# sasg/cilium

Hardware: AMD Instinct MI355X
Metric: classified headers/sec (Mpps, whole node) at 100k-prefix ipcache + 16k-ID policy (higher is better)
Workload: dtype u32

## Files before the change

### cilium_amd/csrc/cfc_api.cpp

```cpp
#include <hip/hip_runtime.h>

#include <algorithm>
#include <cerrno>
#include <cstdio>
#include <cstdlib>
#include <cstring>
#include <map>
#include <set>
#include <memory>
#include <mutex>
#include <string>
#include <thread>
#include <unordered_set>
#include <type_traits>
#include <vector>

#include "../../include/cfc.h"
#include "classify.hpp"
#include "selfcut.hpp"
#include "ctmirror.hpp"
#include "flatten.hpp"
#include "maps.hpp"

using namespace cfc;
// ... 1719 lines not shown
    r.ep = ep_lxc;
    r.m = m;
    const size_t tb = nat_sort_tmp_bytes(m);
    const size_t m4 = 4ull * ((m + 3) & ~3u);
    const size_t rows = V6 ? 5 * m4 + m4 : 8 * m4 + 4 * m4 + m4;
    if (r.idx.ensure(4ull * m) || c->nat_tmp.ensure(tb) || r.rows.ensure(rows) ||
        r.outs.ensure(3 * m4 + 2 * m4))
        return -ENOMEM;
    uint32_t *idx = (uint32_t *)r.idx.p;
    if (int rc = nat_sort((const uint32_t *)c->nat_list.p, idx, m, in.n, c->nat_tmp.p, tb, s))
        return rc;
    char *rp = (char *)r.rows.p, *op = (char *)r.outs.p;
    r.o = cfc_out{};
    r.o.verdict = (int32_t *)op;
    r.o.identity = (uint32_t *)(op + m4);
    r.o.notify = out.notify ? (uint32_t *)(op + 2 * m4) : nullptr;
    r.o.action = (uint8_t *)(op + 3 * m4);
    r.o.ct = (uint8_t *)(op + 4 * m4);
    EgressArgs e2 = ea;
    e2.nat_idx = e2.nat_cnt = nullptr;
    e2.sums = nullptr;
    e2.svo = nullptr;
    const int smode = V6 ? CFC_MODE_EGRESS : CFC_MODE_INGRESS;
    const WsLayout wl = ws_layout(m, T, smode, true);
    if (r.ws.ensure(wl.total))
        return -ENOMEM;
    DevTables Th = T;
    Th.ct_sum = nullptr;
    int rc;
    if constexpr (V6) {
        NatHop4 h{};
        h.sa = (uint32_t *)rp;
        h.da = (uint32_t *)(rp + m4);
        h.pt = (uint32_t *)(rp + 2 * m4);
        h.mt = (uint32_t *)(rp + 3 * m4);
        h.hash = T.lb4 ? (uint32_t *)(rp + 4 * m4) : nullptr;
        h.tf = (uint8_t *)(rp + 5 * m4);
        r.h4 = cfc_hdr_v4{h.sa, h.da, h.pt, h.mt, nullptr, h.tf, m, h.hash};
        rc = nat64_gather(in, idx, m, ea.nat_v4, h, s);
        uint32_t nsvo = 0;
        if (!rc && T.lb4) {
            const size_t sb = svc_order_tmp_bytes(m);
            if (c->svo_keys.bytes < 8ull * m || c->svo.bytes < 4ull * m ||
                c->svo_tmp.bytes < sb) {
                (void)hipStreamSynchronize(s);
                if (c->svo_keys.ensure(8ull * m) || c->svo_keys2.ensure(8ull * m) ||
                    c->svo_tmp.ensure(sb) || c->svo.zeros(4ull * m, s))
// ... 10 lines not shown
                e2.svo = (const uint32_t *)c->svo.p;
        }
        if (!rc)
            rc = launch_classify_v4(Th, r.h4, r.o, smode, e2, c->ctr, (uint32_t *)r.ws.p,
                                    c->num_cus, s, nullptr);
        if ((nsvo || (rc && T.lb4)) && c->svo.p &&
            hipMemsetAsync(c->svo.p, 0, 4ull * m, s) != hipSuccess && !rc)
            rc = -EIO;
    } else {
        NatHop6 h{};
        h.sa = (uint4 *)rp;
        h.da = (uint4 *)(rp + 4 * m4);
        h.pt = (uint32_t *)(rp + 8 * m4);
        h.mt = (uint32_t *)(rp + 9 * m4);
        h.mk = (uint32_t *)(rp + 10 * m4);
        h.id = (uint32_t *)(rp + 11 * m4);
        h.tf = (uint8_t *)(rp + 12 * m4);
        r.h6 = cfc_hdr_v6{(const uint8_t *)h.sa, (const uint8_t *)h.da, h.pt, h.mt, h.mk, h.tf,
                          m, nullptr};
        e2.nat_id = h.id;
        const bool egr = mode == CFC_MODE_EGRESS;
        cfc_hdr_v4 gin = in;
        if (egr && (T.lb4 || T.rnat4)) {
            const WsLayout lw = ws_layout(in.n, T, mode, true);
            const uint32_t *a = (const uint32_t *)((const char *)c->ws + lw.lb);
            const uint64_t st = (in.n + 3) & ~3ull;
            gin.saddr = a + 2 * st;
            gin.daddr = a + 3 * st;
        }
        rc = nat46_gather(T, gin, egr ? nullptr : out.identity, ea.seclabel, idx, m,
                          (const uint4 *)c->epoch->ep->nat6.p, h, s);
        if (!rc)
            rc = launch_classify_v6(Th, r.h6, r.o, smode, e2, c->ctr, (uint32_t *)r.ws.p,
                                    c->num_cus, s, nullptr);
    }
    if (!rc)
        rc = nat_scatter(idx, m, r.o, out, !V6 && mode == CFC_MODE_EGRESS, s);
    c->n_nat_hops += m;
    if (rc || !out.ct)
        r.family = 0;
    return rc;
}

struct Launch4 {
    const uint32_t *tr_id = nullptr;
    int operator()(const DevTables &T, const cfc_hdr_v4 &in, const cfc_out &out, int mode,
                   const EgressArgs &E, uint64_t *ctr, uint32_t *ws, int cus, hipStream_t s,
// ... 49 lines not shown
        if (mode == CFC_MODE_EGRESS) {
            auto it = E.ep->nat4.find(ep_lxc);
            ea.nat_v4 = it == E.ep->nat4.end() ? 0u : it->second;
            nat_list = ea.nat_v4 != 0 && in->n;
        }
    } else {
        T.nat46 = mode != CFC_MODE_XDP && E.T.ct4 && E.ep->nat6.p &&
                  (E.ct->n_nat46 || c->nat46_seen);
        nat_list = T.nat46 && in->n;
    }
    if (nat_list) {
        if (c->nat_list.bytes < 4 * in->n) {
            (void)hipStreamSynchronize(s);
            if (c->nat_list.ensure(4 * in->n))
                return -ENOMEM;
        }
        if (c->nat_cnt.ensure(16) || hipMemsetAsync(c->nat_cnt.p, 0, 4, s) != hipSuccess)
            return -ENOMEM;
        ea.nat_idx = (uint32_t *)c->nat_list.p;
        ea.nat_cnt = (uint32_t *)c->nat_cnt.p;
    }
    const WsLayout wl = ws_layout(in->n, E.T, mode,
                                  E.T.ct4 || E.T.ct6 || out->ct || E.T.lb4 || E.T.rnat4 ||
                                      E.T.lb6 || E.T.rnat6);
    const size_t need = wl.total;
    c->last_cls.valid = false;
    if (need > c->ws_bytes) {
        if (c->ws) {
            (void)hipDeviceSynchronize();
            (void)hipFree(c->ws);
        }
        c->ws = nullptr;
        c->ws_bytes = 0;
        if (hipMalloc((void **)&c->ws, need) != hipSuccess)
            return -ENOMEM;
        c->ws_bytes = need;
    }
    if (c->ctr_pending && c->last_stream != s)
        (void)hipStreamWaitEvent(s, c->last_done, 0);
    order_after_launches(c, s);
    uint32_t nsvo = 0;
    if (mode == CFC_MODE_EGRESS && in->n &&
        (std::is_same<Hdr, cfc_hdr_v6>::value ? E.T.lb6 != nullptr : E.T.lb4 != nullptr)) {
        const uint64_t n = in->n;
        const size_t tb = svc_order_tmp_bytes(n);
        if (c->svo_keys.bytes < 8 * n || c->svo.bytes < 4 * n || c->svo_tmp.bytes < tb) {
            (void)hipStreamSynchronize(s);
// ... 2551 lines not shown
```

### cilium_amd/csrc/classify.hip

```cpp
#include <algorithm>
#include <cstdlib>
#include <mutex>
#include <set>
#include <tuple>
#include <vector>

#include "kern_common.hpp"
#ifndef CFC_EXP
#define CFC_EXP 0
#endif

namespace cfc {

namespace {

constexpr int LDS_MET_U64 = 18;
template <int MODE>
constexpr int met_n()
{
    return MODE == CFC_MODE_EGRESS ? 7 : MODE == CFC_MODE_XDP ? 0 : 4;
}
template <int MODE>
constexpr int acc_n()
{
// ... 500 lines not shown
    p.lxc_slots = (T.lxc4 && T.lxc4_lds) ? T.lxc4_mask + 1 : 0;
    p.pf_words = T.pf_bloom ? T.pf_bloom_words : 0;
    p.pol_words = T.pol_bloom ? T.pol_bloom_words : 0;
    p.pol_disp = T.pol_direct ? p.pol_words : 0;
    return p;
}

template <int MODE>
__device__ __forceinline__ void acc_publish(const unsigned long long *s_met,
                                            const CountArgs &C, uint32_t seclabel)
{
    for (uint32_t j = threadIdx.x; j < 2u * acc_n<MODE>(); j += BLOCK) {
        const unsigned long long v = s_met[j];
        if (!v)
            continue;
        const uint32_t k = j >> 1;
        uint64_t *dst = k < (uint32_t)met_n<MODE>()
                            ? C.g_met + met_reason_dir<MODE>(k) * 2
                            : C.g_id + id_index(ID_DIR_INGRESS, seclabel, k - met_n<MODE>());
        atomicAdd((unsigned long long *)dst + (j & 1), v);
    }
}

template <int MODE, int U, bool CT, bool NT, bool OPT, bool LB, int FAST, bool TR = false>
__global__ __launch_bounds__(BLOCK, WAVES_PER_SIMD) void k_classify_v4(
    DevTables T, LdsPlan L, cfc_hdr_v4 in, cfc_out out, EgressArgs E,
    CountArgs C, uint64_t per_block, LbIn LI, const uint32_t *tr_id)
{
    if (FAST) {
        T.tbl24 = T.tbl8 = T.pf_tbl24 = T.pf_tbl8 = nullptr;
        T.l4_shift = 32 - FAST;
        __builtin_assume(T.l4d != nullptr);
        __builtin_assume(T.lxc4 != nullptr);
        if (MODE == CFC_MODE_XDP || MODE == CFC_MODE_FULL)
            __builtin_assume(T.pf_fix != nullptr);
    }
    unsigned long long *s_met = lds_met();
    Lds S;
    S.lxc_off = LDS_MET_U64 / 2;
    const uint32_t pf4 = S.lxc_off + L.lxc_slots;
    const uint32_t pol4 = pf4 + L.pf_words / 4;
    S.pfb_off = 4 * pf4;
    S.polb_off = 4 * pol4;
    S.lxc = FAST || L.lxc_slots != 0;
    S.pfb = FAST || L.pf_words != 0;
    S.polb = FAST || L.pol_words != 0;
// ... 31 lines not shown
        if (out.ct)
            out.ct += start;
    }
    out.verdict += start;
    out.identity += start;
    if (out.notify)
        out.notify += start;
    constexpr bool LBE = LB && MODE == CFC_MODE_EGRESS;
    if (LBE) {
        LI.tda += start;
        LI.tpt += start;
        LI.psa += start;
        LI.fl += start;
    }
    if (LB && out.pkt_saddr) {
        out.pkt_saddr += start;
        out.pkt_daddr += start;
        out.pkt_ports += start;
    }
    if (C.ct)
        C.ct += start;
    if (C.ct2)
        C.ct2 += start;
    if (C.ctr)
        C.ctr += start;
    if (C.ctr2)
        C.ctr2 += start;
    if (C.id)
        C.id += start;
    if (TR)
        tr_id += start;
    MetAcc<acc_n<MODE>()> acc;
    acc.clear();
    uint32_t iter = 0;
    Raw nx[U];
#pragma unroll
    for (int u = 0; u < U; u++)
        r1_issue<OPT, LBE>(in, LI, u * BLOCK + threadIdx.x, end, nx[u]);
    for (uint32_t base = 0; base < end; base += BLOCK * U) {
        Hdr h[U];
#pragma unroll
        for (int u = 0; u < U; u++)
            r1_take(nx[u], base + u * BLOCK + threadIdx.x, end, h[u]);
#pragma unroll
        for (int u = 0; u < U; u++)
            r2_issue<MODE>(T, S, h[u]);
#pragma unroll
        for (int u = 0; u < U; u++)
            r3_identity<MODE, CT, LB, TR>(T, S, E, h[u], tr_id,
                                          min(base + u * BLOCK + threadIdx.x, end - 1));
        const uint32_t nb = base + BLOCK * U;
#pragma unroll
// ... 13 lines not shown
                if (OPT && out.action)
                    sto((uint8_t)h[u].act, out.action, o);
                if (CT && OPT && out.ct)
                    sto((uint8_t)h[u].ct_byte, out.ct, o);
                if (NT)
                    sto_nt((uint32_t)(h[u].ver < 0
                              ? notify_word(MODE, h[u].ver,
                                            EGR && h[u].met1 == mkey<MODE>(DROP_POLICY, METRIC_INGRESS),
                                            h[u].rec.w & 0xFFFF, E.lxc_id)
                              : h[u].evw),
                          out.notify, o4);
                if (CT) {
                    sto_nt(h[u].ct_k1, C.ct, o4);
                    if (EGR)
                        sto_nt(h[u].ct_k2, C.ct2, o4);
                }
                if (LB && out.pkt_saddr) {
                    sto_nt(h[u].psa, out.pkt_saddr, o4);
                    sto_nt(h[u].da, out.pkt_daddr, o4);
                    sto_nt(h[u].ppt, out.pkt_ports, o4);
                }
                if (MODE != CFC_MODE_XDP) {
#if CFC_EXP != 3
                    sto_nt(ctr_key(C, h[u].ctr0, len), C.ctr, o4);
#endif
                    if (EGR)
                        sto_nt(ctr_key(C, h[u].ctr1, len), C.ctr2, o4);
#if CFC_EXP != 3
                    sto_nt(h[u].idw, C.id, o4);
#endif
                }
            }
            if (WL && E.wbits) {
                bool pr;
                const bool w = wl_want<EGR>(h[u].ct_byte, h[u].ver, h[u].mt, h[u].ct_k1,
                                            EGR ? h[u].ct_k2 : NONE, pr);
                const uint64_t wb = __ballot(w && h[u].valid), pb = __ballot(pr && h[u].valid);
                const uint32_t w0 = base + u * BLOCK + (threadIdx.x & ~63u);
                if ((threadIdx.x & 63) == 0 && w0 < end) {
                    E.wbits[(start + w0) >> 6] = wb;
                    E.wprobe[(start + w0) >> 6] = pb;
                }
            }
            if (MODE != CFC_MODE_XDP && E.nat_idx)
                list_append(E.nat_idx, E.nat_cnt, h[u].nat && h[u].valid, (uint32_t)start + i);
            if (MODE != CFC_MODE_XDP && h[u].valid && h[u].id_ovf && h[u].need_pol)
                id_count(C, id_dir, h[u].ident, h[u].drop1, len);
            if (LBE && h[u].valid && h[u].ver == DROP_NO_SERVICE) {
                unsigned long long *m = reinterpret_cast<unsigned long long *>(
                    C.g_met + (uint64_t)(-DROP_NO_SERVICE * METRIC_DIRS + METRIC_EGRESS) * 2);
                atomicAdd(m, 1ull);
                atomicAdd(m + 1, (unsigned long long)len);
            }
#if CFC_EXP != 5
            acc.add(h[u].valid ? h[u].met0 : NONE, len);
#endif
            if (EGR) {
                acc.add(h[u].valid ? h[u].met1 : NONE, len);
                acc.add(h[u].valid && h[u].ev2 ? met_n<MODE>() + h[u].ev2 - 1 : NONE, len);
            }
        }
        if (++iter == 65536 / (2 * U)) {
            acc.flush(s_met);
            iter = 0;
        }
    }
    acc.flush(s_met);
    __syncthreads();
    acc_publish<MODE>(s_met, C, E.seclabel);
}

}

namespace {

struct HistJob {
    const uint32_t *keys;
    uint64_t poff;
    uint32_t lo, cnt;
    uint32_t kind;
    uint32_t packed;
};
constexpr int HIST_JOBS_MAX = 12;
struct HistJobs {
    HistJob j[HIST_JOBS_MAX];
};
constexpr uint64_t SLICE_MAX = 1ull << 31;

__device__ __forceinline__ unsigned long long *hist_dst(const HistJob &jb, uint32_t key,
                                                        uint64_t *g_ctr, uint64_t *g_id,
                                                        uint32_t id_dir)
{
    return reinterpret_cast<unsigned long long *>(
        jb.kind == 0 ? g_ctr + 2ull * key : g_id + id_index(id_dir, key >> 1, key & 1));
}

struct HistLds {
    uint32_t *ek, *ec, *ew;
    uint32_t *s;
};
__device__ __forceinline__ HistLds hist_lds()
{
    uint32_t *b = reinterpret_cast<uint32_t *>(cfc_smem);
    return HistLds{b, b + HIST_ESC_SLOTS, b + 2 * HIST_ESC_SLOTS, b + 3 * HIST_ESC_SLOTS};
// ... 35 lines not shown
    uint32_t h = fmix32(a.r) & (HIST_ESC_SLOTS - 1);
    for (int p = 0; p < 8; p++) {
        uint32_t cur = L.ek[h];
        if (cur == NONE) {
            cur = atomicCAS(&L.ek[h], NONE, a.r);
            if (cur == NONE)
                cur = a.r;
        }
        if (cur == a.r) {
            if (carry)
                atomicAdd(&L.ec[h], carry);
            if (wrap)
                atomicAdd(&L.ew[h], wrap);
            return;
        }
        h = (h + 1) & (HIST_ESC_SLOTS - 1);
    }
    unsigned long long *d = hist_dst(jb, jb.lo + a.r, g_ctr, g_id, id_dir);
    atomicAdd(d, (unsigned long long)HistSlot::esc_packets(carry, wrap));
    if (carry)
        atomicAdd(d + 1, (unsigned long long)HistSlot::esc_bytes(carry));
}

__global__ __launch_bounds__(BLOCK) void k_hist(HistJobs J, const uint32_t *meta,
                                                uint64_t n, uint64_t per_block,
                                                uint32_t *partial, uint64_t *g_ctr,
                                                uint64_t *g_id, uint32_t id_dir)
{
    const HistJob jb = J.j[blockIdx.y];
    const HistLds L = hist_lds();
    uint32_t *s = L.s;
    for (uint32_t j = threadIdx.x; j < HIST_ESC_SLOTS; j += BLOCK) {
        L.ek[j] = NONE;
        L.ec[j] = 0;
        L.ew[j] = 0;
    }
    for (uint32_t j = threadIdx.x; j < jb.cnt; j += BLOCK)
        s[j] = 0;
    __syncthreads();
    const uint64_t start = (uint64_t)blockIdx.x * per_block;
    const uint64_t end = min(n, start + per_block);
    const uint64_t end4 = start + ((end - start) & ~3ull);
    const bool meta16 = (reinterpret_cast<uintptr_t>(meta) & 15) == 0;
    auto load = [&](uint64_t i, uint4 &w, uint4 &m) {
        w = make_uint4(KEY_NONE, KEY_NONE, KEY_NONE, KEY_NONE);
        m = make_uint4(0, 0, 0, 0);
        if (i >= end4)
            return;
        w = ld_nt4(jb.keys + i);
        if (!jb.packed) {
            if (meta16) {
                m = ld_nt4(meta + i);
            } else {
                m.x = meta[i];
                m.y = meta[i + 1];
                m.z = meta[i + 2];
                m.w = meta[i + 3];
            }
        }
    };
    const uint64_t i0 = start + 4 * threadIdx.x;
    uint4 w0, m0, w1, m1;
    load(i0, w0, m0);
    load(i0 + 4 * BLOCK, w1, m1);
// ... 742 lines not shown
    hipLaunchKernelGGL(k_patch16, dim3((unsigned)((n + 255) / 256)), dim3(256), 0, s, rec, n);
    return hipGetLastError() == hipSuccess ? 0 : -5;
}

int launch_add_u64(uint64_t *dst, const uint64_t *src, uint64_t n,
                   hipStream_t s)
{
    if (!n)
        return 0;
    hipLaunchKernelGGL(k_add_u64, dim3((unsigned)((n + 255) / 256)), dim3(256),
                       0, s, dst, src, n);
    return hipGetLastError() == hipSuccess ? 0 : -5;
}

uint32_t ctp_buckets(const DevTables &T)
{
    if (getenv("CFC_ACC_PER_SLICE"))
        return 0;
    const uint64_t slots = (T.ct4 ? T.ct4_mask + 1ull : 0) + (T.ct6 ? T.ct6_mask + 1ull : 0);
    const uint64_t nb = (2 * slots + CTP_BUCKET - 1) / CTP_BUCKET;
    return nb <= CTP_MAX_BUCKETS ? (uint32_t)nb : 0u;
}

WsLayout ws_layout(uint64_t n, const DevTables &T, int mode, bool ct)
{
    WsLayout w{};
    if (n == 0 || mode == CFC_MODE_XDP)
        return w;
    const bool egr = mode == CFC_MODE_EGRESS;
    const size_t a = 4 * ctr_stride(n);
    size_t off = 0;
    w.ctr = off;
    off += a;
    if (egr) {
        w.ctr2 = off;
        off += a;
    }
    w.id = off;
    off += a;
    if (ct) {
        w.ct = off;
        off += a;
        if (egr) {
            w.ct2 = off;
            off += a;
        }
    }
    off = (off + 255) & ~(size_t)255;
    w.partial = off;
    const uint64_t slots = hist_slots(T, mode);
    w.nblk = hist_slices(n, slots);
    off += 4ull * slots * w.nblk;
    const uint32_t nbuck = ctp_buckets(T);
    if (ct && T.ct_st && nbuck) {
        const uint64_t per = acc_slice(n);
        const uint32_t nblk = (uint32_t)((n + per - 1) / per);
        w.ctp_nv = nblk * (egr ? 2u : 1u);
        w.ctp_nbuck = nbuck;
        w.ctp_nco = (nbuck + ACC_FINE - 1) / ACC_FINE;
        const uint64_t cap = (uint64_t)w.ctp_nv * ACC_RCAP;
        const uint64_t nc = (uint64_t)w.ctp_nco * w.ctp_nv * ACC_SLICE_CHUNKS;
        w.ctp_g2 = (uint32_t)((cap + ACC_CHUNK - 1) / ACC_CHUNK + w.ctp_nco);
// ... 2 lines not shown
            const size_t at = off;
            off += bytes;
            return at;
        };
        w.ctp_rec = take(8 * cap);
        w.ctp_recA = take(8 * cap);
        w.ctp_rcnt = take(4ull * w.ctp_nv);
        w.ctp_cnt = take(4 * nc);
        w.ctp_off = take(4 * nc + 4);
        w.ctp_bsum = take(4 * ((nc + 4 * BLOCK - 1) / (4 * BLOCK)) + 4);
        w.ctp_plan = take(4ull * (2 * w.ctp_nco + 2));
        w.ctp_fo = take(4ull * w.ctp_g2 * (ACC_FINE + 1));
    }
    if (egr && (T.lb4 || T.rnat4)) {
        off = (off + 255) & ~(size_t)255;
        w.lb = off;
        off += 6 * a;
    }
    w.total = off;
    return w;
}

CountArgs count_args(uint32_t *ws, const WsLayout &w, const DevTables &T,
                     uint64_t *g_met, int mode, bool ct)
{
    CountArgs C{};
    char *b = reinterpret_cast<char *>(ws);
    if (w.total) {
        C.ctr = reinterpret_cast<uint32_t *>(b + w.ctr);
        C.ctr2 = mode == CFC_MODE_EGRESS ? reinterpret_cast<uint32_t *>(b + w.ctr2) : nullptr;
        C.id = reinterpret_cast<uint32_t *>(b + w.id);
        C.ct = ct ? reinterpret_cast<uint32_t *>(b + w.ct) : nullptr;
        C.ct2 = ct && mode == CFC_MODE_EGRESS ? reinterpret_cast<uint32_t *>(b + w.ct2)
                                              : nullptr;
    }
    C.g_met = g_met;
    C.g_id = g_met + METRIC_U64;
    C.ctr_packed = T.n_ctr < PACK_MAX;
    return C;
}

int launch_classify_v4(const DevTables &T, const cfc_hdr_v4 &in,
                       const cfc_out &out, int mode, const EgressArgs &E,
                       uint64_t *g_ctr, uint32_t *ws, int num_cus, hipStream_t s,
                       const LaunchTiming *tm, const uint32_t *tr_id)
{
    if (in.n == 0)
        return 0;
    if (classify_lds_bytes(T) > LDS_PER_WG)
        return -22;
    const uint64_t step = (uint64_t)BLOCK * CFC_UNROLL;
    const uint64_t nwg = (uint64_t)num_cus * CFC_WG_PER_CU;
    uint64_t per_block = (in.n + nwg - 1) / nwg;
    per_block = (per_block + step - 1) / step * step;
    per_block = std::min<uint64_t>(per_block, (1ull << 30) / step * step);
    const uint32_t grid = (uint32_t)((in.n + per_block - 1) / per_block);
    if (tm)
        (void)hipEventRecord(tm->ev[0], s);
    const bool lb = (T.lb4 || T.rnat4) && mode != CFC_MODE_XDP;
    const bool ct = T.ct4 || out.ct || lb;
    const WsLayout w = ws_layout(in.n, T, mode, ct);
    const CountArgs C = count_args(ws, w, T, g_ctr + 2ull * T.n_ctr, mode, ct);
    cfc_hdr_v4 hin = in;
    LbIn li{};
    if (lb && mode == CFC_MODE_EGRESS) {
        uint32_t *a = reinterpret_cast<uint32_t *>(reinterpret_cast<char *>(ws) + w.lb);
        const uint64_t st = ctr_stride(in.n);
        LbArgs A{in.saddr, in.daddr, in.ports, in.meta, in.hash, in.n, E.lxc_id,
                 E.ct_owner, a, a + st, a + 2 * st, a + 3 * st, a + 4 * st, a + 5 * st, E.svo};
        if (int rc = launch_lb4_egress(T, A, s))
            return rc;
        li = LbIn{A.tda, A.tpt, A.psa, A.fl};
        hin.daddr = A.pda;
        hin.ports = A.ppt;
    } else if (out.pkt_saddr && !lb) {
        if (hipMemcpyAsync(out.pkt_saddr, in.saddr, 4 * in.n, hipMemcpyDeviceToDevice, s) ||
            hipMemcpyAsync(out.pkt_daddr, in.daddr, 4 * in.n, hipMemcpyDeviceToDevice, s) ||
            hipMemcpyAsync(out.pkt_ports, in.ports, 4 * in.n, hipMemcpyDeviceToDevice, s))
            return -5;
    }
    const LbIn *lbp = lb ? &li : nullptr;
#define CFC_LAUNCH(M)                                                        \
    (ct ? launch_mode<M, true>(T, hin, out, E, C, grid, per_block, s, lbp, tr_id)   \
        : launch_mode<M, false>(T, hin, out, E, C, grid, per_block, s, lbp, tr_id))
    switch (mode) {
    case CFC_MODE_INGRESS: CFC_LAUNCH(CFC_MODE_INGRESS); break;
    case CFC_MODE_EGRESS: CFC_LAUNCH(CFC_MODE_EGRESS); break;
    case CFC_MODE_XDP:
        launch_mode<CFC_MODE_XDP, false>(T, hin, out, E, C, grid, per_block, s, nullptr, nullptr);
        break;
    case CFC_MODE_FULL: CFC_LAUNCH(CFC_MODE_FULL); break;
    default: return -22;
    }
#undef CFC_LAUNCH
    if (tm)
        (void)hipEventRecord(tm->ev[1], s);
    const bool sums = launch_counters(T, in.meta, in.tcp_flags, in.n, mode, ws, g_ctr, s, ct);
    if (E.sums)
        *E.sums = sums;
    if (tm)
        (void)hipEventRecord(tm->ev[2], s);
    hipError_t e = hipGetLastError();
    return e == hipSuccess ? 0 : -5;
}

bool launch_counters(const DevTables &T, const uint32_t *meta, const uint8_t *tf, uint64_t n,
                     int mode, uint32_t *ws, uint64_t *g_ctr, hipStream_t s,
                     bool ct)
{
    bool sums = false;
    if (!n || mode == CFC_MODE_XDP)
        return sums;
    const WsLayout w = ws_layout(n, T, mode, ct);
    const CountArgs C = count_args(ws, w, T, g_ctr + 2ull * T.n_ctr, mode, ct);
    if (ct && T.ct_st && w.ctp_nv) {
        char *b = reinterpret_cast<char *>(ws);
        uint64_t *rec = reinterpret_cast<uint64_t *>(b + w.ctp_rec);
        uint64_t *recA = reinterpret_cast<uint64_t *>(b + w.ctp_recA);
        uint32_t *rcnt = reinterpret_cast<uint32_t *>(b + w.ctp_rcnt);
        uint32_t *cnt = reinterpret_cast<uint32_t *>(b + w.ctp_cnt);
        uint32_t *off = reinterpret_cast<uint32_t *>(b + w.ctp_off);
        uint32_t *bsum = reinterpret_cast<uint32_t *>(b + w.ctp_bsum);
        uint32_t *plan = reinterpret_cast<uint32_t *>(b + w.ctp_plan);
        uint32_t *fo = reinterpret_cast<uint32_t *>(b + w.ctp_fo);
        const uint64_t per = acc_slice(n);
        const uint32_t nblk = (uint32_t)((n + per - 1) / per);
        const uint32_t nch = w.ctp_nv * ACC_SLICE_CHUNKS;
        const uint64_t nc = (uint64_t)w.ctp_nco * nch;
        const uint32_t nsb = (uint32_t)((nc + 4 * BLOCK - 1) / (4 * BLOCK));
        const bool vec = ((uintptr_t)meta & 15) == 0 && (!T.ct_sum || ((uintptr_t)tf & 3) == 0);
        const void *agg = vec ? (const void *)k_acc_agg<true> : (const void *)k_acc_agg<false>;
        set_lds_limit(agg, (int)ACC_AGG_LDS);
        if (vec)
            hipLaunchKernelGGL(k_acc_agg<true>, dim3(nblk, mode == CFC_MODE_EGRESS ? 2 : 1),
                               dim3(BLOCK), ACC_AGG_LDS, s, C.ct, C.ct2, meta,
                               T.ct_sum ? tf : nullptr, T.ct_sum != nullptr, n,
                               w.ctp_nco, rec, rcnt, cnt, per);
// ... 4 lines not shown
                               w.ctp_nco, rec, rcnt, cnt, per);
        hipLaunchKernelGGL(k_scan_local, dim3(nsb), dim3(BLOCK), 0, s, cnt, off, nc, bsum);
        hipLaunchKernelGGL(k_scan_top, dim3(1), dim3(BLOCK), 0, s, bsum, nsb, off + nc);
        hipLaunchKernelGGL(k_scan_add, dim3(nsb), dim3(BLOCK), 0, s, off, nc, bsum);
        set_lds_limit((const void *)k_acc_part1, (int)ACC_SORT_LDS);
        hipLaunchKernelGGL(k_acc_part1, dim3(nch), dim3(BLOCK), ACC_SORT_LDS, s, rec, rcnt,
                           off, nch, w.ctp_nco, recA);
        hipLaunchKernelGGL(k_acc_plan, dim3(1), dim3(64), 0, s, off, nch, w.ctp_nco, plan);
        set_lds_limit((const void *)k_acc_part2, (int)ACC_SORT_LDS);
        hipLaunchKernelGGL(k_acc_part2, dim3(w.ctp_g2), dim3(BLOCK), ACC_SORT_LDS, s, recA,
                           plan, w.ctp_nco, rec, fo);
        set_lds_limit((const void *)k_acc_reduce, (int)ACC_RED_LDS);
        hipLaunchKernelGGL(k_acc_reduce, dim3(w.ctp_nbuck), dim3(BLOCK), ACC_RED_LDS, s, rec,
                           plan, fo, w.ctp_nco, T.ct_st, T.ct_sum);
        sums = T.ct_sum != nullptr;
    } else if (ct && T.ct_st) {
        set_lds_limit((const void *)k_ct_count, (int)CT_LDS_BYTES);
        const uint32_t nblk = (uint32_t)((n + COUNT_PER_BLOCK - 1) / COUNT_PER_BLOCK);
        hipLaunchKernelGGL(k_ct_count, dim3(nblk, mode == CFC_MODE_EGRESS ? 2 : 1),
                           dim3(BLOCK), CT_LDS_BYTES, s, C.ct, C.ct2, meta, n, T.ct_st);
    }
    std::vector<HistJob> jobs;
    uint64_t poff = 0;
    auto add_jobs = [&](const uint32_t *keys, uint32_t nkeys, uint32_t kind,
                        uint32_t packed) {
        for (uint32_t lo = 0; lo < nkeys; lo += HIST_RANGE) {
            HistJob j{keys, poff, lo, std::min(HIST_RANGE, nkeys - lo), kind, packed};
            poff += (uint64_t)w.nblk * j.cnt;
            jobs.push_back(j);
        }
    };
    add_jobs(C.ctr, T.n_ctr, 0, C.ctr_packed);
    if (mode == CFC_MODE_EGRESS)
        add_jobs(C.ctr2, T.n_ctr, 0, C.ctr_packed);
    for (uint32_t r = 0; r < ID_RANGES; r++) {
        if (!((T.id_cover >> r) & 1))
            continue;
        const uint32_t lo = 2 * r * ID_RANGE;
        HistJob j{C.id, poff, lo, std::min(2 * ID_RANGE, 2 * ID_PACK_LIMIT - lo), 1, 1};
        poff += (uint64_t)w.nblk * j.cnt;
        jobs.push_back(j);
    }
    if (jobs.empty())
        return sums;
    uint32_t *partial = reinterpret_cast<uint32_t *>(reinterpret_cast<char *>(ws) + w.partial);
    const uint64_t per_block = hist_per_block(n, w.nblk);
    set_lds_limit((const void *)k_hist, (int)(HIST_ESC_BYTES + 4 * HIST_RANGE));
    const uint32_t id_dir = mode == CFC_MODE_EGRESS ? ID_DIR_EGRESS : ID_DIR_INGRESS;
    for (size_t a = 0; a < jobs.size(); a += HIST_JOBS_MAX) {
        HistJobs J{};
        const uint32_t nj = (uint32_t)std::min<size_t>(HIST_JOBS_MAX, jobs.size() - a);
        uint32_t cmax = 0;
        for (uint32_t k = 0; k < nj; k++) {
            J.j[k] = jobs[a + k];
            cmax = std::max(cmax, J.j[k].cnt);
        }
        hipLaunchKernelGGL(k_hist, dim3(w.nblk, nj), dim3(BLOCK),
                           HIST_ESC_BYTES + 4ull * cmax, s, J, meta, n, per_block, partial,
                           g_ctr, C.g_id, id_dir);
        hipLaunchKernelGGL(k_hist_reduce,
                           dim3((cmax + 255) / 256, nj, (w.nblk + REDUCE_ROWS - 1) / REDUCE_ROWS),
                           dim3(256), 0, s, J, partial, w.nblk, g_ctr, C.g_id, id_dir);
    }
    return sums;
}

}
```

### cilium_amd/csrc/classify.hpp

```cpp
#pragma once
#include <hip/hip_runtime.h>
#include <stdint.h>

#include <algorithm>
#include <cerrno>

#include "../../include/cfc.h"
#include "layout.h"

namespace cfc {

struct EgressArgs {
    uint32_t lxc_id;
    uint32_t seclabel;
    uint32_t pol_base;
    uint32_t pol_mask;
    uint32_t ct_owner;
    uint32_t nat_v4;
    uint32_t *nat_idx, *nat_cnt;
    const uint32_t *nat_id;
    bool *sums;
    const uint32_t *svo;
    uint64_t *wbits, *wprobe;
};
// ... 27 lines not shown
    __host__ __device__ static uint64_t packets(uint32_t slot) { return slot >> BY; }
    __host__ __device__ static uint64_t bytes(uint32_t slot) { return slot & BYMASK; }
    __host__ __device__ static uint64_t esc_packets(uint64_t carries, uint64_t wraps)
    {
        return (wraps << PK) - carries;
    }
    __host__ __device__ static uint64_t esc_bytes(uint64_t carries) { return carries << BY; }
};

constexpr uint32_t ID_SLOTS = 65537;
constexpr uint64_t ID_U64 = 2ull * ID_SLOTS * 2 * 2;
__host__ __device__ inline uint64_t id_index(uint32_t dir, uint32_t ident,
                                             uint32_t drop)
{
    const uint32_t s = ident < ID_SLOTS - 1 ? ident : ID_SLOTS - 1;
    return (((uint64_t)dir * ID_SLOTS + s) * 2 + drop) * 2;
}
constexpr uint32_t ID_DIR_INGRESS = 0, ID_DIR_EGRESS = 1;
constexpr uint32_t ID_RANGE = HIST_RANGE / 2;
constexpr uint32_t ID_PACK_LIMIT = 32768;
constexpr uint32_t ID_RANGES = (ID_PACK_LIMIT + ID_RANGE - 1) / ID_RANGE;
__host__ __device__ inline uint32_t id_range_of(uint32_t ident) { return ident / ID_RANGE; }

struct CountArgs {
    uint32_t *ctr;
    uint32_t *ctr2;
    uint32_t *id;
    uint32_t *ct;
    uint32_t *ct2;
    uint64_t *g_met;
    uint64_t *g_id;
    uint32_t ctr_packed;
};

struct LaunchTiming {
    hipEvent_t ev[3];
    bool v6;
};

struct WsLayout {
    size_t ctr, ctr2, id, ct, ct2, partial, total;
    uint32_t nblk;
    size_t ctp_rec, ctp_recA, ctp_rcnt, ctp_cnt, ctp_off, ctp_bsum, ctp_plan, ctp_fo;
    uint32_t ctp_nv, ctp_nbuck, ctp_nco, ctp_g2;
    size_t lb;
};
WsLayout ws_layout(uint64_t n, const DevTables &T, int mode, bool ct);
CountArgs count_args(uint32_t *ws, const WsLayout &w, const DevTables &T,
                     uint64_t *g_met, int mode, bool ct);
size_t classify_lds_bytes(const DevTables &T);

struct alignas(16) Patch16 {
    uint32_t val[4];
    uint64_t dst;
    uint64_t pad;
};
int launch_patch16(const Patch16 *rec, uint64_t n, hipStream_t stream);

struct CtLog {
    uint32_t x, y, w;
    uint32_t now;
    uint32_t dirlen;
    uint32_t sec;
    uint32_t seq, order;
    uint32_t lbw, slave;
};
constexpr uint32_t CTLOG_NAT46 = 1u << 30;
struct CtLog6 {
    uint4 x, y;
    uint32_t w, now, dirlen, sec, seq, order, rev, slave;
};
struct LbRec4 {
// ... 276 lines not shown

struct RevArgs {
    const void *sa, *da;
    const uint32_t *pt, *mt, *mk;
    void *osa;
    uint32_t *opt, *omk, *oid;
    unsigned long long *hits;
    uint64_t n;
};
int launch_revproxy(const DevTables &T, const RevTables &R, const RevArgs &A, bool v6,
                    int num_cus, hipStream_t s);

int launch_add_u64(uint64_t *dst, const uint64_t *src, uint64_t n,
                   hipStream_t stream);

int launch_classify_v4(const DevTables &T, const cfc_hdr_v4 &in,
                       const cfc_out &out, int mode, const EgressArgs &E,
                       uint64_t *g_ctr, uint32_t *workspace, int num_cus,
                       hipStream_t stream, const LaunchTiming *timing = nullptr,
                       const uint32_t *tr_id = nullptr);

bool launch_counters(const DevTables &T, const uint32_t *meta, const uint8_t *tf, uint64_t n,
                     int mode, uint32_t *workspace, uint64_t *g_ctr,
                     hipStream_t stream, bool ct);

int launch_classify_v6(const DevTables &T, const cfc_hdr_v6 &in,
                       const cfc_out &out, int mode, const EgressArgs &E,
                       uint64_t *g_ctr, uint32_t *workspace, int num_cus,
                       hipStream_t stream, const LaunchTiming *timing = nullptr,
                       const uint32_t *tr_id = nullptr);

void set_lds_limit(const void *kernel, int bytes);

struct NotifyArgs {
    const uint32_t *notify;
    const int32_t *verdict;
    const uint32_t *identity;
    const uint32_t *meta;
    const uint32_t *ports;
    const uint32_t *saddr;
    const uint32_t *daddr;
    const uint32_t *hash;
    uint64_t n;
    int family;
    int mode;
    uint32_t own_seclabel;
    const uint2 *ep_info;
// ... 44 lines not shown
```

### cilium_amd/csrc/classify6.hip

```cpp
#include "kern_common.hpp"

namespace cfc {

namespace {

constexpr int DROP_INVALID_EXTHDR = -156, DROP_FRAG_NOSUPPORT = -157;
constexpr int VERDICT_PUNT = CFC_VERDICT_PUNT;

constexpr int LDS_MET6_U64 = 22;
template <int MODE>
constexpr int met6_n()
{
    return MODE == CFC_MODE_EGRESS ? 9 : MODE == CFC_MODE_XDP ? 0 : 6;
}
template <int MODE>
constexpr int acc6_n()
{
    return met6_n<MODE>() + (MODE == CFC_MODE_EGRESS ? 2 : 0);
}
template <int MODE>
__host__ __device__ constexpr uint32_t met6_reason_dir(int k)
{
    constexpr uint32_t eg[9][2] = {{0, 2},   {132, 2}, {133, 2}, {137, 2}, {140, 2},
                                   {156, 2}, {157, 2}, {0, 1},   {133, 1}};
// ... 617 lines not shown
                       const LaunchTiming *tm, const uint32_t *tr_id)
{
    if (in.n == 0)
        return 0;
    if (lds_plan6(T).bytes() > LDS_PER_WG)
        return -22;
    if ((reinterpret_cast<uintptr_t>(in.saddr) | reinterpret_cast<uintptr_t>(in.daddr)) & 15)
        return -22;
    if (out.pkt_saddr && ((reinterpret_cast<uintptr_t>(out.pkt_saddr) |
                           reinterpret_cast<uintptr_t>(out.pkt_daddr)) & 15))
        return -22;
    if (out.pkt_saddr && mode == CFC_MODE_XDP &&
        (hipMemcpyAsync(out.pkt_saddr, in.saddr, 16 * in.n, hipMemcpyDeviceToDevice, s) ||
         hipMemcpyAsync(out.pkt_daddr, in.daddr, 16 * in.n, hipMemcpyDeviceToDevice, s) ||
         hipMemcpyAsync(out.pkt_ports, in.ports, 4 * in.n, hipMemcpyDeviceToDevice, s)))
        return -5;
    const uint64_t nwg = (uint64_t)num_cus * CFC_WG_PER_CU;
    uint64_t per_block = (in.n + nwg - 1) / nwg;
    per_block = (per_block + BLOCK - 1) / BLOCK * BLOCK;
    const uint32_t grid = (uint32_t)((in.n + per_block - 1) / per_block);
    if (tm)
        (void)hipEventRecord(tm->ev[0], s);
    const bool ct = T.ct6 || out.ct;
    const WsLayout w = ws_layout(in.n, T, mode, ct);
    const CountArgs C = count_args(ws, w, T, g_ctr + 2ull * T.n_ctr, mode, ct);
#define CFC_LAUNCH6(M)                                                         \
    (ct ? launch_mode6<M, true>(T, in, out, E, C, grid, per_block, s, tr_id)   \
        : launch_mode6<M, false>(T, in, out, E, C, grid, per_block, s, tr_id))
    switch (mode) {
    case CFC_MODE_INGRESS: CFC_LAUNCH6(CFC_MODE_INGRESS); break;
    case CFC_MODE_EGRESS: CFC_LAUNCH6(CFC_MODE_EGRESS); break;
    case CFC_MODE_XDP: launch_mode6<CFC_MODE_XDP, false>(T, in, out, E, C, grid, per_block, s, nullptr); break;
    case CFC_MODE_FULL: CFC_LAUNCH6(CFC_MODE_FULL); break;
    default: return -22;
    }
#undef CFC_LAUNCH6
    if (tm)
        (void)hipEventRecord(tm->ev[1], s);
    const bool sums = launch_counters(T, in.meta, in.tcp_flags, in.n, mode, ws, g_ctr, s, ct);
    if (E.sums)
        *E.sums = sums;
    if (tm)
        (void)hipEventRecord(tm->ev[2], s);
    return hipGetLastError() == hipSuccess ? 0 : -5;
}

}
```

Baseline: 61890.

## Compact per-wave counter and identity keys to shrink histogram input

In the v4 classify kernel, each wave now uses a ballot to compact valid counter and identity keys into its own region, instead of writing one key slot per packet. It also stores a per-wave count, which the histogram kernel uses to read only the live keys. The aim is to cut the store and load traffic spent on KEY_NONE entries in the workspace. In exchange it adds ballot and mbcnt work to the hot loop, changes the workspace layout and hist job setup, and shifts the per-block sizing of the hist kernel.

```diff
diff --git a/cilium_amd/csrc/cfc_api.cpp b/cilium_amd/csrc/cfc_api.cpp
--- a/cilium_amd/csrc/cfc_api.cpp
+++ b/cilium_amd/csrc/cfc_api.cpp
@@ -1765,7 +1765,7 @@
     e2.sums = nullptr;
     e2.svo = nullptr;
     const int smode = V6 ? CFC_MODE_EGRESS : CFC_MODE_INGRESS;
-    const WsLayout wl = ws_layout(m, T, smode, true);
+    const WsLayout wl = ws_layout(m, T, smode, true, c->num_cus);
     if (r.ws.ensure(wl.total))
         return -ENOMEM;
     DevTables Th = T;
@@ -1822,7 +1822,7 @@
         const bool egr = mode == CFC_MODE_EGRESS;
         cfc_hdr_v4 gin = in;
         if (egr && (T.lb4 || T.rnat4)) {
-            const WsLayout lw = ws_layout(in.n, T, mode, true);
+            const WsLayout lw = ws_layout(in.n, T, mode, true, c->num_cus);
             const uint32_t *a = (const uint32_t *)((const char *)c->ws + lw.lb);
             const uint64_t st = (in.n + 3) & ~3ull;
             gin.saddr = a + 2 * st;
@@ -1918,7 +1918,8 @@
     }
     const WsLayout wl = ws_layout(in->n, E.T, mode,
                                   E.T.ct4 || E.T.ct6 || out->ct || E.T.lb4 || E.T.rnat4 ||
-                                      E.T.lb6 || E.T.rnat6);
+                                      E.T.lb6 || E.T.rnat6,
+                                  c->num_cus);
     const size_t need = wl.total;
     c->last_cls.valid = false;
     if (need > c->ws_bytes) {
diff --git a/cilium_amd/csrc/classify.hip b/cilium_amd/csrc/classify.hip
--- a/cilium_amd/csrc/classify.hip
+++ b/cilium_amd/csrc/classify.hip
@@ -546,6 +546,32 @@
     }
 }
 
+#ifndef CFC_KEY_NT
+#define CFC_KEY_NT 1
+#endif
+#ifndef CFC_KEYS_COMPACT
+#define CFC_KEYS_COMPACT KEYS_CTR
+#endif
+__device__ __forceinline__ uint32_t key_wave()
+{
+    return __builtin_amdgcn_readfirstlane(threadIdx.x >> 6);
+}
+__device__ __forceinline__ void key_append(uint32_t key, bool valid, uint32_t *region,
+                                           uint32_t &cur)
+{
+    const bool live = valid && key != KEY_NONE;
+    const uint64_t m = __ballot(live);
+    const uint32_t rank = __builtin_amdgcn_mbcnt_hi(
+        (uint32_t)(m >> 32), __builtin_amdgcn_mbcnt_lo((uint32_t)m, 0u));
+    if (live) {
+        if (CFC_KEY_NT)
+            sto_nt(key, region, (cur + rank) << 2);
+        else
+            sto(key, region, (cur + rank) << 2);
+    }
+    cur += (uint32_t)__popcll(m);
+}
+
 template <int MODE, int U, bool CT, bool NT, bool OPT, bool LB, int FAST, bool TR = false>
 __global__ __launch_bounds__(BLOCK, WAVES_PER_SIMD) void k_classify_v4(
     DevTables T, LdsPlan L, cfc_hdr_v4 in, cfc_out out, EgressArgs E,
@@ -623,12 +649,18 @@
         C.ct += start;
     if (C.ct2)
         C.ct2 += start;
-    if (C.ctr)
-        C.ctr += start;
-    if (C.ctr2)
-        C.ctr2 += start;
-    if (C.id)
-        C.id += start;
+    constexpr bool KC = (CFC_KEYS_COMPACT & KEYS_ID) != 0;
+    const bool kc_ctr = (CFC_KEYS_COMPACT & KEYS_CTR) && C.ctr_packed;
+    uint32_t kn_ctr = 0, kn_ctr2 = 0, kn_id = 0;
+    {
+        const uint32_t at = key_wave() * key_regions_grid(gridDim.x, per_block).cap;
+        if (C.ctr)
+            C.ctr += start + (kc_ctr ? at : 0u);
+        if (C.ctr2)
+            C.ctr2 += start + (kc_ctr ? at : 0u);
+        if (C.id)
+            C.id += start + (KC ? at : 0u);
+    }
     if (TR)
         tr_id += start;
     MetAcc<acc_n<MODE>()> acc;
@@ -688,15 +720,27 @@
                 }
                 if (MODE != CFC_MODE_XDP) {
 #if CFC_EXP != 3
-                    sto_nt(ctr_key(C, h[u].ctr0, len), C.ctr, o4);
-#endif
-                    if (EGR)
-                        sto_nt(ctr_key(C, h[u].ctr1, len), C.ctr2, o4);
-#if CFC_EXP != 3
-                    sto_nt(h[u].idw, C.id, o4);
+                    if (!kc_ctr) {
+                        sto_nt(ctr_key(C, h[u].ctr0, len), C.ctr, o4);
+                        if (EGR)
+                            sto_nt(ctr_key(C, h[u].ctr1, len), C.ctr2, o4);
+                    }
+                    if (!KC)
+                        sto_nt(h[u].idw, C.id, o4);
 #endif
                 }
             }
+#if CFC_EXP != 3
+            if (MODE != CFC_MODE_XDP) {
+                if (kc_ctr) {
+                    key_append(ctr_key(C, h[u].ctr0, len), h[u].valid, C.ctr, kn_ctr);
+                    if (EGR)
+                        key_append(ctr_key(C, h[u].ctr1, len), h[u].valid, C.ctr2, kn_ctr2);
+                }
+                if (KC)
+                    key_append(h[u].idw, h[u].valid, C.id, kn_id);
+            }
+#endif
             if (WL && E.wbits) {
                 bool pr;
                 const bool w = wl_want<EGR>(h[u].ct_byte, h[u].ver, h[u].mt, h[u].ct_k1,
@@ -732,6 +776,20 @@
         }
     }
     acc.flush(s_met);
+    if (CFC_KEYS_COMPACT && MODE != CFC_MODE_XDP && (threadIdx.x & 63) == 0) {
+        const uint32_t wave = key_wave();
+        const uint64_t to_counts =
+            (uint64_t)(gridDim.x - blockIdx.x) * per_block -
+            (uint64_t)wave * key_regions_grid(gridDim.x, per_block).cap +
+            (uint64_t)blockIdx.x * KEY_WAVES + wave;
+        if (kc_ctr) {
+            C.ctr[to_counts] = kn_ctr;
+            if (EGR)
+                C.ctr2[to_counts] = kn_ctr2;
+        }
+        if (KC)
+            C.id[to_counts] = kn_id;
+    }
     __syncthreads();
     acc_publish<MODE>(s_met, C, E.seclabel);
 }
@@ -746,6 +804,9 @@
     uint32_t lo, cnt;
     uint32_t kind;
     uint32_t packed;
+    uint32_t compact, cap;
+    const uint32_t *counts;
+    uint64_t n, per_block;
 };
 constexpr int HIST_JOBS_MAX = 12;
 struct HistJobs {
@@ -827,8 +888,49 @@
         atomicAdd(d + 1, (unsigned long long)HistSlot::esc_bytes(carry));
 }
 
+__device__ __forceinline__ void hist_compact(const HistLds &L, const HistJob &jb,
+                                             uint64_t start, uint64_t stop, uint64_t *g_ctr,
+                                             uint64_t *g_id, uint32_t id_dir)
+{
+    if (start >= stop)
+        return;
+    const uint32_t wave = __builtin_amdgcn_readfirstlane(threadIdx.x >> 6);
+    const uint32_t lane4 = 4 * (threadIdx.x & 63);
+    const uint32_t r1 = (uint32_t)((stop + jb.cap - 1) / jb.cap);
+    uint32_t r = (uint32_t)(start / jb.cap) + wave;
+    uint32_t cnt = r < r1 ? jb.counts[r] : 0u;
+    while (r < r1) {
+        const uint32_t rn = r + KEY_WAVES;
+        const uint32_t cnt_n = rn < r1 ? jb.counts[rn] : 0u;
+        const uint64_t rb = (uint64_t)r * jb.cap;
+        const uint64_t lo = max(rb, start), hi = min(rb + min(cnt, jb.cap), stop);
+        if (lo < hi) {
+            const uint32_t len = (uint32_t)(hi - lo), last = (len - 1) & ~3u;
+            const uint32_t *k = jb.keys + lo;
+            uint4 w0 = ld_nt4(k + min(lane4, last));
+            uint4 w1 = ld_nt4(k + min(lane4 + 256, last));
+            for (uint32_t o = lane4, b = 0; b < len; b += 256, o += 256) {
+                const uint4 w2 = ld_nt4(k + min(o + 512, last));
+                const HistAdd a0 = hist_add(L.s, jb, o < len ? w0.x : KEY_NONE, 0u);
+                const HistAdd a1 = hist_add(L.s, jb, o + 1 < len ? w0.y : KEY_NONE, 0u);
+                const HistAdd a2 = hist_add(L.s, jb, o + 2 < len ? w0.z : KEY_NONE, 0u);
+                const HistAdd a3 = hist_add(L.s, jb, o + 3 < len ? w0.w : KEY_NONE, 0u);
+                if (hist_spills(a0) | hist_spills(a1) | hist_spills(a2) | hist_spills(a3)) {
+                    hist_escape(L, jb, a0, g_ctr, g_id, id_dir);
+                    hist_escape(L, jb, a1, g_ctr, g_id, id_dir);
+                    hist_escape(L, jb, a2, g_ctr, g_id, id_dir);
+                    hist_escape(L, jb, a3, g_ctr, g_id, id_dir);
+                }
+                w0 = w1;
+                w1 = w2;
+            }
+        }
+        r = rn;
+        cnt = cnt_n;
+    }
+}
+
 __global__ __launch_bounds__(BLOCK) void k_hist(HistJobs J, const uint32_t *meta,
-                                                uint64_t n, uint64_t per_block,
                                                 uint32_t *partial, uint64_t *g_ctr,
                                                 uint64_t *g_id, uint32_t id_dir)
 {
@@ -843,8 +945,11 @@
     for (uint32_t j = threadIdx.x; j < jb.cnt; j += BLOCK)
         s[j] = 0;
     __syncthreads();
-    const uint64_t start = (uint64_t)blockIdx.x * per_block;
-    const uint64_t end = min(n, start + per_block);
+    const uint64_t start = (uint64_t)blockIdx.x * jb.per_block;
+    const uint64_t stop = max(start, min(jb.n, start + jb.per_block));
+    if (jb.compact)
+        hist_compact(L, jb, start, stop, g_ctr, g_id, id_dir);
+    const uint64_t end = jb.compact ? start : stop;
     const uint64_t end4 = start + ((end - start) & ~3ull);
     const bool meta16 = (reinterpret_cast<uintptr_t>(meta) & 15) == 0;
     auto load = [&](uint64_t i, uint4 &w, uint4 &m) {
@@ -1633,22 +1738,25 @@
     return nb <= CTP_MAX_BUCKETS ? (uint32_t)nb : 0u;
 }
 
-WsLayout ws_layout(uint64_t n, const DevTables &T, int mode, bool ct)
+WsLayout ws_layout(uint64_t n, const DevTables &T, int mode, bool ct, int num_cus)
 {
     WsLayout w{};
     if (n == 0 || mode == CFC_MODE_XDP)
         return w;
     const bool egr = mode == CFC_MODE_EGRESS;
     const size_t a = 4 * ctr_stride(n);
+    w.key_pb = key_per_block(n, (uint64_t)std::max(num_cus, 1) * CFC_WG_PER_CU,
+                             (uint64_t)BLOCK * CFC_UNROLL);
+    const size_t ka = std::max<size_t>(a, 4 * key_regions(n, w.key_pb).words());
     size_t off = 0;
     w.ctr = off;
-    off += a;
+    off += ka;
     if (egr) {
         w.ctr2 = off;
-        off += a;
+        off += ka;
     }
     w.id = off;
-    off += a;
+    off += ka;
     if (ct) {
         w.ct = off;
         off += a;
@@ -1697,7 +1805,7 @@
 }
 
 CountArgs count_args(uint32_t *ws, const WsLayout &w, const DevTables &T,
-                     uint64_t *g_met, int mode, bool ct)
+                     uint64_t *g_met, int mode, bool ct, bool v4)
 {
     CountArgs C{};
     char *b = reinterpret_cast<char *>(ws);
@@ -1712,6 +1820,8 @@
     C.g_met = g_met;
     C.g_id = g_met + METRIC_U64;
     C.ctr_packed = T.n_ctr < PACK_MAX;
+    if (v4 && w.total)
+        C.compact = CFC_KEYS_COMPACT & (KEYS_ID | (C.ctr_packed ? KEYS_CTR : 0u));
     return C;
 }
 
@@ -1724,18 +1834,15 @@
         return 0;
     if (classify_lds_bytes(T) > LDS_PER_WG)
         return -22;
-    const uint64_t step = (uint64_t)BLOCK * CFC_UNROLL;
-    const uint64_t nwg = (uint64_t)num_cus * CFC_WG_PER_CU;
-    uint64_t per_block = (in.n + nwg - 1) / nwg;
-    per_block = (per_block + step - 1) / step * step;
-    per_block = std::min<uint64_t>(per_block, (1ull << 30) / step * step);
+    const uint64_t per_block = key_per_block(in.n, (uint64_t)std::max(num_cus, 1) * CFC_WG_PER_CU,
+                                             (uint64_t)BLOCK * CFC_UNROLL);
     const uint32_t grid = (uint32_t)((in.n + per_block - 1) / per_block);
     if (tm)
         (void)hipEventRecord(tm->ev[0], s);
     const bool lb = (T.lb4 || T.rnat4) && mode != CFC_MODE_XDP;
     const bool ct = T.ct4 || out.ct || lb;
-    const WsLayout w = ws_layout(in.n, T, mode, ct);
-    const CountArgs C = count_args(ws, w, T, g_ctr + 2ull * T.n_ctr, mode, ct);
+    const WsLayout w = ws_layout(in.n, T, mode, ct, num_cus);
+    const CountArgs C = count_args(ws, w, T, g_ctr + 2ull * T.n_ctr, mode, ct, true);
     cfc_hdr_v4 hin = in;
     LbIn li{};
     if (lb && mode == CFC_MODE_EGRESS) {
@@ -1770,7 +1877,8 @@
 #undef CFC_LAUNCH
     if (tm)
         (void)hipEventRecord(tm->ev[1], s);
-    const bool sums = launch_counters(T, in.meta, in.tcp_flags, in.n, mode, ws, g_ctr, s, ct);
+    const bool sums = launch_counters(T, in.meta, in.tcp_flags, in.n, mode, ws, g_ctr, s, ct,
+                                      C, w);
     if (E.sums)
         *E.sums = sums;
     if (tm)
@@ -1781,13 +1889,11 @@
 
 bool launch_counters(const DevTables &T, const uint32_t *meta, const uint8_t *tf, uint64_t n,
                      int mode, uint32_t *ws, uint64_t *g_ctr, hipStream_t s,
-                     bool ct)
+                     bool ct, const CountArgs &C, const WsLayout &w)
 {
     bool sums = false;
     if (!n || mode == CFC_MODE_XDP)
         return sums;
-    const WsLayout w = ws_layout(n, T, mode, ct);
-    const CountArgs C = count_args(ws, w, T, g_ctr + 2ull * T.n_ctr, mode, ct);
     if (ct && T.ct_st && w.ctp_nv) {
         char *b = reinterpret_cast<char *>(ws);
         uint64_t *rec = reinterpret_cast<uint64_t *>(b + w.ctp_rec);
@@ -1838,29 +1944,42 @@
     }
     std::vector<HistJob> jobs;
     uint64_t poff = 0;
-    auto add_jobs = [&](const uint32_t *keys, uint32_t nkeys, uint32_t kind,
-                        uint32_t packed) {
-        for (uint32_t lo = 0; lo < nkeys; lo += HIST_RANGE) {
-            HistJob j{keys, poff, lo, std::min(HIST_RANGE, nkeys - lo), kind, packed};
-            poff += (uint64_t)w.nblk * j.cnt;
-            jobs.push_back(j);
-        }
+    const KeyRegions KG = key_regions(n, w.key_pb);
+    auto job = [&](const uint32_t *keys, uint32_t lo, uint32_t cnt, uint32_t kind,
+                   uint32_t packed, bool compact) {
+        HistJob j{};
+        j.keys = keys;
+        j.poff = poff;
+        j.lo = lo;
+        j.cnt = cnt;
+        j.kind = kind;
+        j.packed = packed;
+        j.compact = compact;
+        j.cap = compact ? KG.cap : 0u;
+        j.counts = compact ? keys + KG.counts() : nullptr;
+        j.n = compact ? KG.extent : n;
+        j.per_block = hist_per_block(j.n, w.nblk);
+        poff += (uint64_t)w.nblk * j.cnt;
+        jobs.push_back(j);
     };
-    add_jobs(C.ctr, T.n_ctr, 0, C.ctr_packed);
+    auto add_jobs = [&](const uint32_t *keys, uint32_t nkeys) {
+        for (uint32_t lo = 0; lo < nkeys; lo += HIST_RANGE)
+            job(keys, lo, std::min(HIST_RANGE, nkeys - lo), 0, C.ctr_packed,
+                (C.compact & KEYS_CTR) != 0);
+    };
+    add_jobs(C.ctr, T.n_ctr);
     if (mode == CFC_MODE_EGRESS)
-        add_jobs(C.ctr2, T.n_ctr, 0, C.ctr_packed);
+        add_jobs(C.ctr2, T.n_ctr);
     for (uint32_t r = 0; r < ID_RANGES; r++) {
         if (!((T.id_cover >> r) & 1))
             continue;
         const uint32_t lo = 2 * r * ID_RANGE;
-        HistJob j{C.id, poff, lo, std::min(2 * ID_RANGE, 2 * ID_PACK_LIMIT - lo), 1, 1};
-        poff += (uint64_t)w.nblk * j.cnt;
-        jobs.push_back(j);
+        job(C.id, lo, std::min(2 * ID_RANGE, 2 * ID_PACK_LIMIT - lo), 1, 1,
+            (C.compact & KEYS_ID) != 0);
     }
     if (jobs.empty())
         return sums;
     uint32_t *partial = reinterpret_cast<uint32_t *>(reinterpret_cast<char *>(ws) + w.partial);
-    const uint64_t per_block = hist_per_block(n, w.nblk);
     set_lds_limit((const void *)k_hist, (int)(HIST_ESC_BYTES + 4 * HIST_RANGE));
     const uint32_t id_dir = mode == CFC_MODE_EGRESS ? ID_DIR_EGRESS : ID_DIR_INGRESS;
     for (size_t a = 0; a < jobs.size(); a += HIST_JOBS_MAX) {
@@ -1872,8 +1991,8 @@
             cmax = std::max(cmax, J.j[k].cnt);
         }
         hipLaunchKernelGGL(k_hist, dim3(w.nblk, nj), dim3(BLOCK),
-                           HIST_ESC_BYTES + 4ull * cmax, s, J, meta, n, per_block, partial,
-                           g_ctr, C.g_id, id_dir);
+                           HIST_ESC_BYTES + 4ull * cmax, s, J, meta, partial, g_ctr, C.g_id,
+                           id_dir);
         hipLaunchKernelGGL(k_hist_reduce,
                            dim3((cmax + 255) / 256, nj, (w.nblk + REDUCE_ROWS - 1) / REDUCE_ROWS),
                            dim3(256), 0, s, J, partial, w.nblk, g_ctr, C.g_id, id_dir);
diff --git a/cilium_amd/csrc/classify.hpp b/cilium_amd/csrc/classify.hpp
--- a/cilium_amd/csrc/classify.hpp
+++ b/cilium_amd/csrc/classify.hpp
@@ -73,6 +73,35 @@
 constexpr uint32_t ID_RANGES = (ID_PACK_LIMIT + ID_RANGE - 1) / ID_RANGE;
 __host__ __device__ inline uint32_t id_range_of(uint32_t ident) { return ident / ID_RANGE; }
 
+constexpr uint32_t KEY_WAVES = BLOCK / 64;
+struct KeyRegions {
+    uint64_t extent;
+    uint32_t cap;
+    uint32_t regions;
+    __host__ __device__ uint64_t base(uint32_t r) const { return (uint64_t)r * cap; }
+    __host__ __device__ uint64_t counts() const { return extent; }
+    __host__ __device__ uint64_t words() const { return extent + ((regions + 3u) & ~3u); }
+};
+__host__ __device__ inline KeyRegions key_regions_grid(uint64_t grid, uint64_t per_block)
+{
+    KeyRegions g;
+    g.extent = grid * per_block;
+    g.cap = (uint32_t)(per_block / KEY_WAVES);
+    g.regions = (uint32_t)(grid * KEY_WAVES);
+    return g;
+}
+__host__ __device__ inline KeyRegions key_regions(uint64_t n, uint64_t per_block)
+{
+    return key_regions_grid((n + per_block - 1) / per_block, per_block);
+}
+__host__ __device__ inline uint64_t key_per_block(uint64_t n, uint64_t nwg, uint64_t step)
+{
+    uint64_t per_block = (n + nwg - 1) / nwg;
+    per_block = (per_block + step - 1) / step * step;
+    const uint64_t top = (1ull << 30) / step * step;
+    return per_block < top ? per_block : top;
+}
+
 struct CountArgs {
     uint32_t *ctr;
     uint32_t *ctr2;
@@ -82,7 +111,9 @@
     uint64_t *g_met;
     uint64_t *g_id;
     uint32_t ctr_packed;
-};
+    uint32_t compact;
+};
+constexpr uint32_t KEYS_CTR = 1, KEYS_ID = 2;
 
 struct LaunchTiming {
     hipEvent_t ev[3];
@@ -92,13 +123,14 @@
 struct WsLayout {
     size_t ctr, ctr2, id, ct, ct2, partial, total;
     uint32_t nblk;
+    uint64_t key_pb;
     size_t ctp_rec, ctp_recA, ctp_rcnt, ctp_cnt, ctp_off, ctp_bsum, ctp_plan, ctp_fo;
     uint32_t ctp_nv, ctp_nbuck, ctp_nco, ctp_g2;
     size_t lb;
 };
-WsLayout ws_layout(uint64_t n, const DevTables &T, int mode, bool ct);
+WsLayout ws_layout(uint64_t n, const DevTables &T, int mode, bool ct, int num_cus);
 CountArgs count_args(uint32_t *ws, const WsLayout &w, const DevTables &T,
-                     uint64_t *g_met, int mode, bool ct);
+                     uint64_t *g_met, int mode, bool ct, bool v4);
 size_t classify_lds_bytes(const DevTables &T);
 
 struct alignas(16) Patch16 {
@@ -421,7 +453,7 @@
 
 bool launch_counters(const DevTables &T, const uint32_t *meta, const uint8_t *tf, uint64_t n,
                      int mode, uint32_t *workspace, uint64_t *g_ctr,
-                     hipStream_t stream, bool ct);
+                     hipStream_t stream, bool ct, const CountArgs &C, const WsLayout &w);
 
 int launch_classify_v6(const DevTables &T, const cfc_hdr_v6 &in,
                        const cfc_out &out, int mode, const EgressArgs &E,
diff --git a/cilium_amd/csrc/classify6.hip b/cilium_amd/csrc/classify6.hip
--- a/cilium_amd/csrc/classify6.hip
+++ b/cilium_amd/csrc/classify6.hip
@@ -663,8 +663,8 @@
     if (tm)
         (void)hipEventRecord(tm->ev[0], s);
     const bool ct = T.ct6 || out.ct;
-    const WsLayout w = ws_layout(in.n, T, mode, ct);
-    const CountArgs C = count_args(ws, w, T, g_ctr + 2ull * T.n_ctr, mode, ct);
+    const WsLayout w = ws_layout(in.n, T, mode, ct, num_cus);
+    const CountArgs C = count_args(ws, w, T, g_ctr + 2ull * T.n_ctr, mode, ct, false);
 #define CFC_LAUNCH6(M)                                                         \
     (ct ? launch_mode6<M, true>(T, in, out, E, C, grid, per_block, s, tr_id)   \
         : launch_mode6<M, false>(T, in, out, E, C, grid, per_block, s, tr_id))
@@ -678,7 +678,8 @@
 #undef CFC_LAUNCH6
     if (tm)
         (void)hipEventRecord(tm->ev[1], s);
-    const bool sums = launch_counters(T, in.meta, in.tcp_flags, in.n, mode, ws, g_ctr, s, ct);
+    const bool sums = launch_counters(T, in.meta, in.tcp_flags, in.n, mode, ws, g_ctr, s, ct,
+                                      C, w);
     if (E.sums)
         *E.sums = sums;
     if (tm)
```

Result: faster. 64800 (median of 6 runs) (+4.7%).
